# Bluear7878/Remote-Sensing-Vision-Language-Diffusion-Model

Measured on AMD Instinct MI355X. Metric: 512px x8 SR images/sec @50 steps, higher is better.
Workload: dtype f16 / bf16 MFMA operands as hi + lo pairs and triples, f32 accumulation and f32 residual streams (Stage 1: f16 tensors x f16 weight pairs; Stage 2: rsvld_amd.ops.UNET_POLICY; config.precision) -- the composition inside 1e-3 of the reference's CPU path (config.tolerance)

## Files before the change

### remote-sensing-vision-language-diffusion-model_amd/csrc/attention.hip

```cpp
#include "rsvld_common.h"
#include <type_traits>
#include <utility>

namespace {

struct AttnArgs {
    const void* q;
    const void* k;
    const void* v;
    void* out;
    int B, heads, Nq, Nk, D;
    int64_t q_bs, q_ts, k_bs, k_ts, v_bs, v_ts, o_bs, o_ts;
    float scale_log2e;
    unsigned long long* dbg;
};

typedef const __attribute__((address_space(1))) void* gptr_t;
typedef __attribute__((address_space(3))) void* lptr_t;

template <typename F, int... I> __device__ __forceinline__ void static_for_impl(F&& f, std::integer_sequence<int, I...>) {
    (f(std::integral_constant<int, I>{}), ...);
}
template <int N, typename F> __device__ __forceinline__ void static_for(F&& f) {
    static_for_impl(f, std::make_integer_sequence<int, N>{});
}

constexpr float A5_DEFER_LOG2 = 8.0f;

#ifndef A5B_KEYWRAP
#define A5B_KEYWRAP 0
#endif
#ifndef A5B_ABL
#define A5B_ABL 0
#endif
constexpr int A5B_TILE = 32 * 1024;
constexpr int A5B_SMEM = 4 * A5B_TILE;
constexpr int A5B_SMEM_SH = 3 * A5B_TILE;
__host__ __device__ constexpr int a5b_f(int r) { return ((r & 3) << 2) | ((r >> 2) & 3); }
typedef short s16x4 __attribute__((__vector_size__(4 * sizeof(short))));
__device__ __forceinline__ float a5b_halfwave_max(float mx) { return fmaxf(mx, __shfl_xor(mx, 32)); }

template <typename T, bool SH>
__global__ __launch_bounds__(256) void attn_d512b_kernel(AttnArgs p, int keys_per_split, float* part_o, float* part_ml) {
    constexpr int D = 512;
    typedef typename Mfma<T>::v8 v8;
    typedef typename Mfma<T>::v4 v4;
    extern __shared__ __attribute__((aligned(16))) char smem[];

    const int tid = threadIdx.x, lane = tid & 63, w = tid >> 6;
    const int l31 = lane & 31, lh = lane >> 5;
    const int q0 = blockIdx.x * 128 + w * 32;
    const int split = blockIdx.y, nsplit = gridDim.y;
    const int b = blockIdx.z / p.heads, h = blockIdx.z % p.heads;
    const int k_begin = split * keys_per_split;
    const int k_end = min(p.Nk, k_begin + keys_per_split);
    const int nt = (k_end - k_begin + 31) >> 5;
    const T* Qb = (const T*)p.q + (int64_t)b * p.q_bs + (int64_t)h * D;
    const T* Kb = (const T*)p.k + (int64_t)b * p.k_bs + (int64_t)h * D;
    const T* Vb = (const T*)p.v + (int64_t)b * p.v_bs + (int64_t)h * D;

    const int wu = __builtin_amdgcn_readfirstlane(w);
    const uint32_t lds0 = (uint32_t)(uintptr_t)(lptr_t)smem;
    bool abl_dma_on = true;
    auto dma_one = [&](const char* base, uint32_t voff, uint32_t dst) {
        if ((A5B_ABL & 4) && !abl_dma_on) return;
        asm volatile("s_mov_b32 m0, %1\n\ts_nop 0\n\tglobal_load_lds_dwordx4 %0, %2" : : "v"(voff), "s"(dst), "s"(base) : "memory", "m0");
    };
    const int64_t k_rowb = p.k_ts * (int64_t)sizeof(T), v_rowb = p.v_ts * (int64_t)sizeof(T);
    uint32_t kvo[8], vvo[8];
#pragma unroll
    for (int i = 0; i < 8; ++i) {
        kvo[i] = (uint32_t)(i * k_rowb) + (uint32_t)((lane ^ (SH ? a5b_f((wu * 8 + i) & 15) : ((wu * 8 + i) & 15))) << 4);
        vvo[i] = (uint32_t)(i * v_rowb) + (uint32_t)((lane ^ ((i & 3) << 2)) << 4);
    }
    const char* k_tile0 = (const char*)(Kb + (int64_t)(k_begin + wu * 8) * p.k_ts);
    const char* v_tile0 = (const char*)(Vb + (int64_t)(k_begin + wu * 8) * p.v_ts);
    auto dma_kb = [&](int t, int buf, int i) {
        const int r = wu * 8 + i;
        const uint32_t dst = lds0 + buf * A5B_TILE + r * 1024;
        if (k_begin + t * 32 + 32 <= p.Nk) {
            dma_one(k_tile0 + (int64_t)t * 32 * k_rowb, kvo[i], dst);
        } else {
            const int key = min(k_begin + t * 32 + r, p.Nk - 1);
            dma_one((const char*)(Kb + (int64_t)key * p.k_ts), (uint32_t)((lane ^ (SH ? a5b_f(r & 15) : (r & 15))) << 4), dst);
        }
    };
    auto dma_k = [&](int t, int i) { dma_kb(t, t & 1, i); };
    auto dma_v = [&](int t, int i) {
        const int r = wu * 8 + i;
        const uint32_t dst = lds0 + (2 + (t & 1)) * A5B_TILE + r * 1024;
        if (k_begin + t * 32 + 32 <= p.Nk) {
            dma_one(v_tile0 + (int64_t)t * 32 * v_rowb, vvo[i], dst);
        } else {
            const int key = min(k_begin + t * 32 + r, p.Nk - 1);
            dma_one((const char*)(Vb + (int64_t)key * p.v_ts), (uint32_t)((lane ^ ((i & 3) << 2)) << 4), dst);
        }
    };
    auto tw = [](int t) { return A5B_KEYWRAP > 0 ? (t & (A5B_KEYWRAP - 1)) : t; };
    auto dma_kb_fast = [&](int t, int buf, int i) { dma_one(k_tile0 + (int64_t)tw(t) * 32 * k_rowb, kvo[i], lds0 + buf * A5B_TILE + (wu * 8 + i) * 1024); };
    auto dma_k_fast = [&](int t, int i) { dma_kb_fast(t, t & 1, i); };
    auto dma_v_fast = [&](int t, int i) { dma_one(v_tile0 + (int64_t)tw(t) * 32 * v_rowb, vvo[i], lds0 + (2 + (t & 1)) * A5B_TILE + (wu * 8 + i) * 1024); };
    if constexpr (SH) {
#pragma unroll
        for (int i = 0; i < 8; ++i) dma_kb(0, 0, i);
        if (nt > 1) {
#pragma unroll
            for (int i = 0; i < 8; ++i) dma_kb(1, 1, i);
        }
        if (A5B_ABL & 4) {
            if (nt > 2) {
#pragma unroll
                for (int i = 0; i < 8; ++i) dma_kb(2, 2, i);
            }
            abl_dma_on = false;
        }
    } else {
#pragma unroll
    for (int i = 0; i < 8; ++i) { dma_k(0, i); dma_v(0, i); }
    if (nt > 1) {
#pragma unroll
        for (int i = 0; i < 8; ++i) dma_k(1, i);
    }
    }
    if (!SH && (A5B_ABL & 4)) {
        if (nt > 1) {
#pragma unroll
            for (int i = 0; i < 8; ++i) dma_v(1, i);
        }
        abl_dma_on = false;
    }

    const int qrow = q0 + l31;
    v8 qf[32];
#pragma unroll
    for (int ks = 0; ks < 32; ++ks) {
        u32x4 v = {0u, 0u, 0u, 0u};
        if (qrow < p.Nq) v = *(const u32x4*)(Qb + (int64_t)qrow * p.q_ts + ks * 16 + lh * 8);
        qf[ks] = __builtin_bit_cast(v8, v);
    }
    f32x16 oacc[16];
#pragma unroll
    for (int dt = 0; dt < 16; ++dt)
#pragma unroll
        for (int r = 0; r < 16; ++r) oacc[dt][r] = 0.f;
    float m_run = -INFINITY, l_run = 0.f;

    int kbase[8];
#pragma unroll
    for (int c = 0; c < 8; ++c) kbase[c] = l31 * 1024 + (((2 * c + lh) ^ (SH ? a5b_f(l31 & 15) : (l31 & 15))) << 4);
    int vbase[4];
    {
        const int qq = (lane >> 2) & 3, pp = lane & 3, g1 = (lane >> 4) & 1;
#pragma unroll
        for (int f = 0; f < 4; ++f)
            vbase[f] = SH ? (4 * lh + qq) * 1024 + ((f ^ qq) << 6) + (((2 * g1 + (pp >> 1)) ^ lh) << 4) + ((pp & 1) << 3)
                          : 2 * A5B_TILE + (4 * lh + qq) * 1024 + ((f ^ qq) << 6) + ((2 * g1 + (pp >> 1)) << 4) + ((pp & 1) << 3);
    }

    asm volatile("s_waitcnt vmcnt(0)" ::: "memory");
    __syncthreads();

    constexpr int KD = 6;
    static_assert(KD == 6, "A5B_CHAIN's prologue issues 6 reads");
    uint32_t ka[8];
    v8 kfr[KD];
#define A5B_KREAD(slot, ks) \
    asm volatile("ds_read_b128 %0, %1 offset:%2" : "=v"(kfr[slot]) : "v"(ka[(ks) & 7]), "i"(((ks) >> 3) * 256))
#define A5B_STEP(NAME, SACC, ks)                                                                                        \
    asm volatile("s_waitcnt lgkmcnt(%3)\n\t" NAME " %0, %1, %2, %0"                                                      \
                 : "+v"(SACC)                                                                                           \
                 : "v"(kfr[(ks) % KD]), "v"(qf[ks]), "i"(KD - 1 < 31 - (ks) ? KD - 1 : 31 - (ks)));                      \
    if constexpr ((ks) + KD < 32 && !(A5B_ABL & 8)) A5B_KREAD((ks) % KD, (ks) + KD)
#define A5B_STEP4(NAME, SACC, k) \
    A5B_STEP(NAME, SACC, k); A5B_STEP(NAME, SACC, (k) + 1); A5B_STEP(NAME, SACC, (k) + 2); A5B_STEP(NAME, SACC, (k) + 3)
#define A5B_CHAIN(NAME, SACC, KBUF, HOOK)                                                                               \
    _Pragma("unroll") for (int c = 0; c < 8; ++c) ka[c] = lds0 + (uint32_t)((KBUF) * A5B_TILE + kbase[c]);              \
    A5B_KREAD(0, 0); A5B_KREAD(1, 1); A5B_KREAD(2, 2); A5B_KREAD(3, 3); A5B_KREAD(4, 4); A5B_KREAD(5, 5);               \
    asm volatile("s_waitcnt lgkmcnt(%3)\n\t" NAME " %0, %1, %2, 0" : "=&v"(SACC) : "v"(kfr[0]), "v"(qf[0]), "i"(KD - 1)); \
    A5B_KREAD(0, KD);                                                                                                   \
    A5B_STEP(NAME, SACC, 1); A5B_STEP(NAME, SACC, 2); A5B_STEP(NAME, SACC, 3); HOOK(0);                                 \
    A5B_STEP4(NAME, SACC, 4); HOOK(1); A5B_STEP4(NAME, SACC, 8); HOOK(2); A5B_STEP4(NAME, SACC, 12); HOOK(3);           \
    A5B_STEP4(NAME, SACC, 16); HOOK(4); A5B_STEP4(NAME, SACC, 20); HOOK(5); A5B_STEP4(NAME, SACC, 24); HOOK(6);         \
    A5B_STEP4(NAME, SACC, 28); HOOK(7)
#define A5B_MFMA_NAME(T_) (__is_same(T_, f16) ? "f16" : "bf16")
#define A5B_NOHOOK(i)

    f32x16 sacc;
    if constexpr (__is_same(T, f16)) {
        A5B_CHAIN("v_mfma_f32_32x32x16_f16", sacc, 0, A5B_NOHOOK);
    } else {
        A5B_CHAIN("v_mfma_f32_32x32x16_bf16", sacc, 0, A5B_NOHOOK);
    }
    asm volatile("s_nop 15\n\ts_nop 3" : "+v"(sacc));
    __syncthreads();

    int b_pv = 0;
    int t = 0;
    f32x16 sacc2;
#define A5B_STEADY 1
#define A5B_PAIR 1
#define dma_kb_s dma_kb_fast
#define dma_k_s dma_k_fast
#define dma_v_s dma_v_fast
    for (; t + 4 < nt;) {
        {
#define S_CUR sacc
#define S_NXT sacc2
#include "attention_d512_body.inc"
#undef S_CUR
#undef S_NXT
        }
        ++t;
        {
#define S_CUR sacc2
#define S_NXT sacc
#include "attention_d512_body.inc"
#undef S_CUR
#undef S_NXT
        }
        ++t;
    }
#undef dma_kb_s
#undef dma_k_s
#undef dma_v_s
#undef A5B_PAIR
#undef A5B_STEADY
    for (; t < nt; ++t) {
#define A5B_PAIR 0
#define S_CUR sacc
#define S_NXT snext
#define A5B_STEADY 0
#define dma_kb_s dma_kb
#define dma_k_s dma_k
#define dma_v_s dma_v
#include "attention_d512_body.inc"
#undef dma_kb_s
#undef dma_k_s
#undef dma_v_s
#undef A5B_STEADY
#undef S_CUR
#undef S_NXT
#undef A5B_PAIR
    }
#undef A5B_NOHOOK
#undef A5B_MFMA_NAME
#undef A5B_CHAIN
#undef A5B_STEP4
#undef A5B_STEP
#undef A5B_KREAD

    const float l_tot = l_run + __shfl_xor(l_run, 32);
    if (qrow >= p.Nq) return;
    const float inv = 1.0f / l_tot;
    if (nsplit == 1) {
        T* Ob = (T*)p.out + (int64_t)b * p.o_bs + (int64_t)h * D + (int64_t)qrow * p.o_ts;
#pragma unroll
        for (int dt = 0; dt < 16; ++dt)
#pragma unroll
            for (int g = 0; g < 4; ++g) {
                v4 o;
#pragma unroll
                for (int e = 0; e < 4; ++e) o[e] = (T)(oacc[dt][4 * g + e] * inv);
                *(v4*)(Ob + dt * 32 + 8 * g + 4 * lh) = o;
            }
    } else {
        const int64_t row = ((int64_t)split * gridDim.z + blockIdx.z) * p.Nq + qrow;
        float* Po = part_o + row * D;
#pragma unroll
        for (int dt = 0; dt < 16; ++dt)
#pragma unroll
            for (int g = 0; g < 4; ++g) {
                f32x4 o;
#pragma unroll
                for (int e = 0; e < 4; ++e) o[e] = oacc[dt][4 * g + e] * inv;
                *(f32x4*)(Po + dt * 32 + 8 * g + 4 * lh) = o;
            }
        if (lh == 0) {
            part_ml[row * 2] = m_run;
            part_ml[row * 2 + 1] = l_tot;
        }
    }
}

template <typename T>
__global__ __launch_bounds__(128) void attn_combine_kernel(AttnArgs p, int nsplit, const float* part_o, const float* part_ml) {
    constexpr int D = 512;
    typedef typename Mfma<T>::v4 v4;
    const int qrow = blockIdx.x, bh = blockIdx.y;
    const int b = bh / p.heads, h = bh % p.heads;
    const int64_t nrows = (int64_t)gridDim.y * p.Nq;
    float mmax = -INFINITY;
    for (int i = 0; i < nsplit; ++i) mmax = fmaxf(mmax, part_ml[((int64_t)i * nrows + (int64_t)bh * p.Nq + qrow) * 2]);
    float wsum = 0.f;
    f32x4 acc = {0.f, 0.f, 0.f, 0.f};
    for (int i = 0; i < nsplit; ++i) {
        const int64_t row = (int64_t)i * nrows + (int64_t)bh * p.Nq + qrow;
        const float wi = part_ml[row * 2 + 1] * __builtin_amdgcn_exp2f(part_ml[row * 2] - mmax);
        const f32x4 o = *(const f32x4*)(part_o + row * D + threadIdx.x * 4);
        acc += o * wi;
        wsum += wi;
    }
    const float inv = 1.0f / wsum;
    v4 o;
#pragma unroll
    for (int e = 0; e < 4; ++e) o[e] = (T)(acc[e] * inv);
    *(v4*)((T*)p.out + (int64_t)b * p.o_bs + (int64_t)h * D + (int64_t)qrow * p.o_ts + threadIdx.x * 4) = o;
}

#include "attention_d512d.inc"

}

namespace {

constexpr int A6B_TILE = 64 * 128;
#ifndef A6B_ABL
#define A6B_ABL 0
#endif
#ifndef A6B_STAMP
#define A6B_STAMP 0
#endif
__device__ __forceinline__ unsigned long long a6b_stamp() {
    unsigned long long t;
    __builtin_amdgcn_sched_barrier(0);
    asm volatile("s_memtime %0\n\ts_waitcnt lgkmcnt(0)" : "=s"(t) :: "memory");
    __builtin_amdgcn_sched_barrier(0);
    return t;
}

__device__ __forceinline__ float a6b_add(float a, float b) { return a + b; }

template <typename T>
__device__ __forceinline__ void a6_store_o(char* wbuf, const f32x16 (&oacc)[2], float inv, int q0, int lane, const AttnArgs& p, int b, int h) {
    typedef typename Mfma<T>::v4 v4;
    const int l31 = lane & 31, lh = lane >> 5;
    T* Ob = (T*)p.out + (int64_t)b * p.o_bs + (int64_t)h * 64;
#pragma unroll
    for (int dt = 0; dt < 2; ++dt)
#pragma unroll
        for (int g = 0; g < 4; ++g) {
            v4 o;
#pragma unroll
            for (int e = 0; e < 4; ++e) o[e] = (T)(oacc[dt][4 * g + e] * inv);
// ... 404 lines not shown
```

### remote-sensing-vision-language-diffusion-model_amd/csrc/attention_d512d.inc

```
constexpr int A5D_P_OFF = 4 * A5B_TILE;
constexpr int A5D_PBUF = 4 * 2 * 64 * 16;
constexpr int A5D_A_OFF = A5D_P_OFF + 2 * A5D_PBUF;
constexpr int A5D_L_OFF = A5D_A_OFF + 2 * 512;
constexpr int A5D_SMEM = A5D_L_OFF + 512;

template <typename T>
__global__ __launch_bounds__(256) void attn_d512d_kernel(AttnArgs p, int keys_per_split, float* part_o, float* part_ml) {
    constexpr int D = 512;
    typedef typename Mfma<T>::v8 v8;
    typedef typename Mfma<T>::v4 v4;
    extern __shared__ __attribute__((aligned(16))) char smem[];

    const int tid = threadIdx.x, lane = tid & 63, w = tid >> 6;
    const int l31 = lane & 31, lh = lane >> 5;
    const int q0 = blockIdx.x * 128 + w * 32;
    const int split = blockIdx.y, nsplit = gridDim.y;
    const int b = blockIdx.z / p.heads, h = blockIdx.z % p.heads;
    const int k_begin = split * keys_per_split;
    const int k_end = min(p.Nk, k_begin + keys_per_split);
    const int nt = (k_end - k_begin + 31) >> 5;
    const T* Qb = (const T*)p.q + (int64_t)b * p.q_bs + (int64_t)h * D;
    const T* Xb = (const T*)p.k + (int64_t)b * p.k_bs + (int64_t)h * D;

    const int wu = __builtin_amdgcn_readfirstlane(w);
    const uint32_t lds0 = (uint32_t)(uintptr_t)(lptr_t)smem;
    auto dma_one = [&](const char* base, uint32_t voff, uint32_t dst) {
        asm volatile("s_mov_b32 m0, %1\n\ts_nop 0\n\tglobal_load_lds_dwordx4 %0, %2" : : "v"(voff), "s"(dst), "s"(base) : "memory", "m0");
    };
    const int64_t x_rowb = p.k_ts * (int64_t)sizeof(T);
    const uint32_t lane16 = (uint32_t)lane << 4;
    const char* x_tile0 = (const char*)(Xb + (int64_t)(k_begin + wu * 8) * p.k_ts);
    auto dma_x = [&](int t, int i) {
        const int r = wu * 8 + i;
        const uint32_t dst = lds0 + (t & 3) * A5B_TILE + r * 1024;
        if (k_begin + t * 32 + 32 <= p.Nk) {
            dma_one(x_tile0 + (int64_t)(t * 32 + i) * x_rowb, lane16 ^ (uint32_t)(a5b_f(r & 15) << 4), dst);
        } else {
            const int key = min(k_begin + t * 32 + r, p.Nk - 1);
            dma_one((const char*)(Xb + (int64_t)key * p.k_ts), lane16 ^ (uint32_t)(a5b_f(r & 15) << 4), dst);
        }
    };
    auto dma_x_fast = [&](int t, int i) {
        const int r = wu * 8 + i;
        dma_one(x_tile0 + (int64_t)(t * 32 + i) * x_rowb, lane16 ^ (uint32_t)(a5b_f(r & 15) << 4), lds0 + (t & 3) * A5B_TILE + r * 1024);
    };
#pragma unroll
    for (int i = 0; i < 8; ++i) dma_x(0, i);
    if (nt > 1) {
#pragma unroll
        for (int i = 0; i < 8; ++i) dma_x(1, i);
    }
    if (nt > 2) {
#pragma unroll
        for (int i = 0; i < 8; ++i) dma_x(2, i);
    }

    const int qrow = q0 + l31;
    v8 qf[32];
#pragma unroll
    for (int ks = 0; ks < 32; ++ks) {
        u32x4 v = {0u, 0u, 0u, 0u};
        if (qrow < p.Nq) v = *(const u32x4*)(Qb + (int64_t)qrow * p.q_ts + ks * 16 + lh * 8);
        qf[ks] = __builtin_bit_cast(v8, v);
    }
    f32x16 oacc[4][4];
#pragma unroll
    for (int dt = 0; dt < 4; ++dt)
#pragma unroll
        for (int j = 0; j < 4; ++j)
#pragma unroll
            for (int r = 0; r < 16; ++r) oacc[dt][j][r] = 0.f;
    float m_run = -INFINITY, l_run = 0.f;

    const uint32_t kb = l31 * 1024 + ((lh ^ a5b_f(l31 & 15)) << 4);
    int vbase[4];
    {
        const int qq = (lane >> 2) & 3, pp = lane & 3, g1 = (lane >> 4) & 1;
#pragma unroll
        for (int f = 0; f < 4; ++f) vbase[f] = (4 * lh + qq) * 1024 + ((f ^ qq) << 6) + (((2 * g1 + (pp >> 1)) ^ lh) << 4) + ((pp & 1) << 3) + wu * 256;
    }
    auto vread = [&](int buf, int f, int s2) {
        const int off = buf * A5B_TILE + vbase[f] + (16 * s2) * 1024;
        const s16x4 lo = __builtin_amdgcn_ds_read_tr16_b64_v4i16((__attribute__((address_space(3))) s16x4*)(smem + off));
        const s16x4 hi = __builtin_amdgcn_ds_read_tr16_b64_v4i16((__attribute__((address_space(3))) s16x4*)(smem + ((off ^ 32) + 8 * 1024)));
        typedef short s16x8 __attribute__((__vector_size__(8 * sizeof(short))));
        return __builtin_bit_cast(v8, (s16x8)__builtin_shufflevector(lo, hi, 0, 1, 2, 3, 4, 5, 6, 7));
    };
    const int p_own = A5D_P_OFF + wu * 2048 + lane * 16, a_own = A5D_A_OFF + l31 * 16 + wu * 4;
    int p_oth[3], a_oth[3];
#pragma unroll
    for (int j = 1; j < 4; ++j) {
        p_oth[j - 1] = A5D_P_OFF + ((wu + j) & 3) * 2048 + lane * 16;
        a_oth[j - 1] = A5D_A_OFF + l31 * 16 + ((wu + j) & 3) * 4;
    }

    asm volatile("s_waitcnt vmcnt(0)" ::: "memory");
    __syncthreads();

    constexpr int KD = 6;
    uint32_t ka[8];
    v8 kfr[KD];
#define A5D_KREAD(slot, ks) \
    asm volatile("ds_read_b128 %0, %1 offset:%2" : "=v"(kfr[slot]) : "v"(ka[(ks) & 7]), "i"(((ks) >> 3) * 256))
#define A5D_STEP(NAME, SACC, ks)                                                                                        \
    asm volatile("s_waitcnt lgkmcnt(%3)\n\t" NAME " %0, %1, %2, %0"                                                      \
                 : "+v"(SACC)                                                                                           \
                 : "v"(kfr[(ks) % KD]), "v"(qf[ks]), "i"(KD - 1 < 31 - (ks) ? KD - 1 : 31 - (ks)));                      \
    if constexpr ((ks) + KD < 32) A5D_KREAD((ks) % KD, (ks) + KD)
#define A5D_STEP4(NAME, SACC, k) \
    A5D_STEP(NAME, SACC, k); A5D_STEP(NAME, SACC, (k) + 1); A5D_STEP(NAME, SACC, (k) + 2); A5D_STEP(NAME, SACC, (k) + 3)
#define A5D_CHAIN(NAME, SACC, KBUF, HOOK)                                                                               \
    _Pragma("unroll") for (int c = 0; c < 8; ++c) ka[c] = lds0 + (((KBUF) * A5B_TILE + kb) ^ (c << 5));         \
    A5D_KREAD(0, 0); A5D_KREAD(1, 1); A5D_KREAD(2, 2); A5D_KREAD(3, 3); A5D_KREAD(4, 4); A5D_KREAD(5, 5);               \
    asm volatile("s_waitcnt lgkmcnt(%3)\n\t" NAME " %0, %1, %2, 0" : "=&v"(SACC) : "v"(kfr[0]), "v"(qf[0]), "i"(KD - 1)); \
    A5D_KREAD(0, KD);                                                                                                   \
    A5D_STEP(NAME, SACC, 1); A5D_STEP(NAME, SACC, 2); A5D_STEP(NAME, SACC, 3); HOOK(0);                                 \
    A5D_STEP4(NAME, SACC, 4); HOOK(1); A5D_STEP4(NAME, SACC, 8); HOOK(2); A5D_STEP4(NAME, SACC, 12); HOOK(3);           \
    A5D_STEP4(NAME, SACC, 16); HOOK(4); A5D_STEP4(NAME, SACC, 20); HOOK(5); A5D_STEP4(NAME, SACC, 24); HOOK(6);         \
    A5D_STEP4(NAME, SACC, 28); HOOK(7)
#define A5D_NOHOOK(i)

    f32x16 sacc;
    if constexpr (__is_same(T, f16)) {
        A5D_CHAIN("v_mfma_f32_32x32x16_f16", sacc, 0, A5D_NOHOOK);
    } else {
        A5D_CHAIN("v_mfma_f32_32x32x16_bf16", sacc, 0, A5D_NOHOOK);
    }
    asm volatile("s_nop 15\n\ts_nop 3" : "+v"(sacc));

    int t = 0;
    f32x16 sacc2;
#define A5D_STEADY 1
#define A5D_PAIR 1
    for (; t + 5 < nt;) {
        {
#define S_CUR sacc
#define S_NXT sacc2
#include "attention_d512d_body.inc"
#undef S_CUR
#undef S_NXT
        }
        ++t;
        {
#define S_CUR sacc2
#define S_NXT sacc
#include "attention_d512d_body.inc"
#undef S_CUR
#undef S_NXT
        }
        ++t;
    }
#undef A5D_PAIR
#undef A5D_STEADY
    for (; t < nt; ++t) {
#define A5D_PAIR 0
#define A5D_STEADY 0
#define S_CUR sacc
#define S_NXT snext
#include "attention_d512d_body.inc"
#undef S_NXT
#undef S_CUR
#undef A5D_STEADY
#undef A5D_PAIR
    }
#undef A5D_NOHOOK
#undef A5D_CHAIN
#undef A5D_STEP4
#undef A5D_STEP
#undef A5D_KREAD

    const float l_tot = l_run + __shfl_xor(l_run, 32);
    *(float*)(smem + A5D_L_OFF + l31 * 16 + wu * 4) = l_tot;
    __syncthreads();
    float inv[4];
    inv[0] = 1.0f / l_tot;
#pragma unroll
    for (int j = 1; j < 4; ++j) inv[j] = 1.0f / *(const float*)(smem + A5D_L_OFF + l31 * 16 + ((wu + j) & 3) * 4);
#pragma unroll
    for (int j = 0; j < 4; ++j) {
        const int qr = blockIdx.x * 128 + ((wu + j) & 3) * 32 + l31;
        if (qr >= p.Nq) continue;
        if (nsplit == 1) {
            T* Ob = (T*)p.out + (int64_t)b * p.o_bs + (int64_t)h * D + (int64_t)qr * p.o_ts + wu * 128;
#pragma unroll
            for (int dt = 0; dt < 4; ++dt)
#pragma unroll
                for (int g = 0; g < 4; ++g) {
                    v4 o;
#pragma unroll
                    for (int e = 0; e < 4; ++e) o[e] = (T)(oacc[dt][j][4 * g + e] * inv[j]);
                    *(v4*)(Ob + dt * 32 + 8 * g + 4 * lh) = o;
                }
        } else {
            const int64_t row = ((int64_t)split * gridDim.z + blockIdx.z) * p.Nq + qr;
            float* Po = part_o + row * D + wu * 128;
#pragma unroll
            for (int dt = 0; dt < 4; ++dt)
#pragma unroll
                for (int g = 0; g < 4; ++g) {
                    f32x4 o;
#pragma unroll
                    for (int e = 0; e < 4; ++e) o[e] = oacc[dt][j][4 * g + e] * inv[j];
                    *(f32x4*)(Po + dt * 32 + 8 * g + 4 * lh) = o;
                }
            if (j == 0 && lh == 0) {
                part_ml[row * 2] = m_run;
                part_ml[row * 2 + 1] = l_tot;
            }
        }
    }
}
```

### remote-sensing-vision-language-diffusion-model_amd/csrc/attention_d512d_body.inc

```
        const bool more = A5D_STEADY ? true : t + 1 < nt;
        const int b_pv = t & 3, pb = (t & 1) * A5D_PBUF, ab = (t & 1) * 512;

        float mx = -INFINITY, alpha = 1.0f, rs = 0.f;
        bool need = false;
        v8 pf[2];
        auto sm = [&](int part) {
            if (part == 0) {
                if (!A5D_STEADY && k_begin + (t + 1) * 32 > k_end) {
#pragma unroll
                    for (int r = 0; r < 16; ++r) {
                        const int kv = k_begin + t * 32 + (r & 3) + 8 * (r >> 2) + 4 * lh;
                        if (kv >= k_end) S_CUR[r] = -INFINITY;
                    }
                }
#pragma unroll
                for (int r = 0; r < 16; ++r) mx = fmaxf(mx, S_CUR[r]);
                asm volatile("" : "+v"(S_CUR), "+v"(mx));
            } else if (part == 1) {
                mx = a5b_halfwave_max(mx) * p.scale_log2e;
                need = mx > m_run + A5_DEFER_LOG2;
                if (need) {
                    alpha = __builtin_amdgcn_exp2f(m_run - mx);
                    m_run = mx;
                }
                asm volatile("" : "+v"(alpha), "+v"(m_run));
            } else if (part >= 2 && part <= 5) {
                const int r0 = 4 * (part - 2);
#pragma unroll
                for (int r = r0; r < r0 + 4; ++r) {
                    S_CUR[r] = __builtin_amdgcn_exp2f(__builtin_fmaf(S_CUR[r], p.scale_log2e, -m_run));
                    rs += S_CUR[r];
                }
                asm volatile("" : "+v"(S_CUR[r0]), "+v"(S_CUR[r0 + 1]), "+v"(S_CUR[r0 + 2]), "+v"(S_CUR[r0 + 3]), "+v"(rs));
            } else if (part == 6) {
                l_run = l_run * alpha + rs;
#pragma unroll
                for (int s2 = 0; s2 < 2; ++s2)
#pragma unroll
                    for (int j = 0; j < 8; ++j) pf[s2][j] = (T)S_CUR[8 * s2 + j];
                asm volatile("" : "+v"(pf[0]), "+v"(pf[1]), "+v"(l_run));
            }
        };
#if !A5D_PAIR
        f32x16 snext;
#endif
        if (more) {
#define A5D_HOOK(i) \
    sm(i);          \
    __builtin_amdgcn_sched_barrier(0)
            if constexpr (__is_same(T, f16)) {
                A5D_CHAIN("v_mfma_f32_32x32x16_f16", S_NXT, ((t + 1) & 3), A5D_HOOK);
            } else {
                A5D_CHAIN("v_mfma_f32_32x32x16_bf16", S_NXT, ((t + 1) & 3), A5D_HOOK);
            }
#undef A5D_HOOK
        } else {
#pragma unroll
            for (int i = 0; i < 7; ++i) sm(i);
        }

        *(v8*)(smem + pb + p_own) = pf[0];
        *(v8*)(smem + pb + p_own + 1024) = pf[1];
        *(float*)(smem + ab + a_own) = alpha;
        v8 vfr[2][4];
#pragma unroll
        for (int s2 = 0; s2 < 2; ++s2)
#pragma unroll
            for (int f = 0; f < 4; ++f) vfr[s2][f] = vread(b_pv, f, s2);
        asm volatile("s_waitcnt vmcnt(0)" ::: "memory");
        __syncthreads();

        v8 pfo[2][3];
        float al[3];
#pragma unroll
        for (int s2 = 0; s2 < 2; ++s2)
#pragma unroll
            for (int j = 0; j < 3; ++j) pfo[s2][j] = *(const v8*)(smem + pb + p_oth[j] + 1024 * s2);
#pragma unroll
        for (int j = 0; j < 3; ++j) al[j] = *(const float*)(smem + ab + a_oth[j]);

#define A5D_RESCALE(J, A)                                                                                                  \
    _Pragma("unroll") for (int dt = 0; dt < 4; ++dt)                                                                       \
    _Pragma("unroll") for (int r = 0; r < 16; ++r) {                                                                       \
        float x = oacc[dt][J][r], tmp;                                                                                     \
        asm volatile("v_accvgpr_read_b32 %1, %0\n\tv_mul_f32 %1, %1, %2\n\ts_nop 0\n\tv_accvgpr_write_b32 %0, %1\n\ts_nop 1" \
                     : "+a"(x), "=&v"(tmp)                                                                                 \
                     : "v"(A));                                                                                            \
        oacc[dt][J][r] = x;                                                                                                \
    }
        if (__builtin_expect(__any(need), 0)) {
            asm volatile("s_nop 15\n\ts_nop 3" ::: "memory");
            A5D_RESCALE(0, alpha)
        }
        __builtin_amdgcn_sched_barrier(0);
#pragma unroll
        for (int s2 = 0; s2 < 2; ++s2)
#pragma unroll
            for (int f = 0; f < 4; ++f) {
                oacc[f][0] = Mfma<T>::mma(vfr[s2][f], pf[s2], oacc[f][0]);
                __builtin_amdgcn_sched_barrier(0);
            }
        if (__builtin_expect(__any(al[0] != 1.0f || al[1] != 1.0f || al[2] != 1.0f), 0)) {
            asm volatile("s_nop 15\n\ts_nop 3" ::: "memory");
            A5D_RESCALE(1, al[0])
            A5D_RESCALE(2, al[1])
            A5D_RESCALE(3, al[2])
        }
#undef A5D_RESCALE
        __builtin_amdgcn_sched_barrier(0);
#pragma unroll
        for (int n = 0; n < 24; ++n) {
            const int s2 = n / 12, f = (n / 3) & 3, j = n % 3;
            oacc[f][j + 1] = Mfma<T>::mma(vfr[s2][f], pfo[s2][j], oacc[f][j + 1]);
            if (n % 3 == 2) {
                if (A5D_STEADY) {
                    dma_x_fast(t + 3, n / 3);
                } else if (t + 3 < nt) {
                    dma_x(t + 3, n / 3);
                }
            }
            __builtin_amdgcn_sched_barrier(0);
        }
#if !A5D_PAIR
        if (more) S_CUR = S_NXT;
#endif
```

Baseline: 0.01348.

## Spread softmax work across QK MFMA chain and hoist max into PV phase

Restructures the online-softmax placement in the d512 attention kernel. The row max and the rescale decision move out of the per-tile softmax and are computed either after the QK chain or interleaved with the own-P PV MFMAs. Exp, conversion and sum work is issued one step at a time after each QK MFMA, and the cross-half max uses permlane32_swap instead of a shuffle. LDS addresses are split into lane and scalar wave parts so they can use SGPR offsets. The aim is to hide softmax VALU latency under MFMA issue, at the cost of more complex scheduling, register pressure, and macro-selected variants.

```diff
diff --git a/remote-sensing-vision-language-diffusion-model_amd/csrc/attention.hip b/remote-sensing-vision-language-diffusion-model_amd/csrc/attention.hip
--- a/remote-sensing-vision-language-diffusion-model_amd/csrc/attention.hip
+++ b/remote-sensing-vision-language-diffusion-model_amd/csrc/attention.hip
@@ -33,12 +33,21 @@
 #ifndef A5B_ABL
 #define A5B_ABL 0
 #endif
+#ifndef A5D_ABL
+#define A5D_ABL 0
+#endif
 constexpr int A5B_TILE = 32 * 1024;
 constexpr int A5B_SMEM = 4 * A5B_TILE;
 constexpr int A5B_SMEM_SH = 3 * A5B_TILE;
 __host__ __device__ constexpr int a5b_f(int r) { return ((r & 3) << 2) | ((r >> 2) & 3); }
 typedef short s16x4 __attribute__((__vector_size__(4 * sizeof(short))));
 __device__ __forceinline__ float a5b_halfwave_max(float mx) { return fmaxf(mx, __shfl_xor(mx, 32)); }
+__device__ __forceinline__ void a5d_halfwave_swap(float mx, float& lo, float& hi) {
+    const uint32_t mb = __builtin_bit_cast(uint32_t, mx);
+    const auto sw = __builtin_amdgcn_permlane32_swap(mb, mb, false, false);
+    lo = __builtin_bit_cast(float, (uint32_t)sw[0]);
+    hi = __builtin_bit_cast(float, (uint32_t)sw[1]);
+}
 
 template <typename T, bool SH>
 __global__ __launch_bounds__(256) void attn_d512b_kernel(AttnArgs p, int keys_per_split, float* part_o, float* part_ml) {
diff --git a/remote-sensing-vision-language-diffusion-model_amd/csrc/attention_d512d.inc b/remote-sensing-vision-language-diffusion-model_amd/csrc/attention_d512d.inc
--- a/remote-sensing-vision-language-diffusion-model_amd/csrc/attention_d512d.inc
+++ b/remote-sensing-vision-language-diffusion-model_amd/csrc/attention_d512d.inc
@@ -1,3 +1,6 @@
+#ifndef A5D_PLACE
+#define A5D_PLACE 7
+#endif
 constexpr int A5D_P_OFF = 4 * A5B_TILE;
 constexpr int A5D_PBUF = 4 * 2 * 64 * 16;
 constexpr int A5D_A_OFF = A5D_P_OFF + 2 * A5D_PBUF;
@@ -86,13 +89,18 @@
         typedef short s16x8 __attribute__((__vector_size__(8 * sizeof(short))));
         return __builtin_bit_cast(v8, (s16x8)__builtin_shufflevector(lo, hi, 0, 1, 2, 3, 4, 5, 6, 7));
     };
-    const int p_own = A5D_P_OFF + wu * 2048 + lane * 16, a_own = A5D_A_OFF + l31 * 16 + wu * 4;
+    const int p_lane = lane * 16, a_lane = l31 * 16;
+    const int p_own = A5D_P_OFF + wu * 2048, a_own = A5D_A_OFF + wu * 4;
     int p_oth[3], a_oth[3];
 #pragma unroll
     for (int j = 1; j < 4; ++j) {
-        p_oth[j - 1] = A5D_P_OFF + ((wu + j) & 3) * 2048 + lane * 16;
-        a_oth[j - 1] = A5D_A_OFF + l31 * 16 + ((wu + j) & 3) * 4;
-    }
+        p_oth[j - 1] = A5D_P_OFF + ((wu + j) & 3) * 2048;
+        a_oth[j - 1] = A5D_A_OFF + ((wu + j) & 3) * 4;
+    }
+    auto xaddr = [&](int lane_part, int wave_part) __attribute__((always_inline)) {
+        asm volatile("" : "+s"(wave_part));
+        return smem + (lane_part + wave_part);
+    };
 
     asm volatile("s_waitcnt vmcnt(0)" ::: "memory");
     __syncthreads();
@@ -102,23 +110,63 @@
     v8 kfr[KD];
 #define A5D_KREAD(slot, ks) \
     asm volatile("ds_read_b128 %0, %1 offset:%2" : "=v"(kfr[slot]) : "v"(ka[(ks) & 7]), "i"(((ks) >> 3) * 256))
-#define A5D_STEP(NAME, SACC, ks)                                                                                        \
+#define A5D_STEP(NAME, SACC, ks, HOOK)                                                                                  \
     asm volatile("s_waitcnt lgkmcnt(%3)\n\t" NAME " %0, %1, %2, %0"                                                      \
                  : "+v"(SACC)                                                                                           \
                  : "v"(kfr[(ks) % KD]), "v"(qf[ks]), "i"(KD - 1 < 31 - (ks) ? KD - 1 : 31 - (ks)));                      \
-    if constexpr ((ks) + KD < 32) A5D_KREAD((ks) % KD, (ks) + KD)
-#define A5D_STEP4(NAME, SACC, k) \
-    A5D_STEP(NAME, SACC, k); A5D_STEP(NAME, SACC, (k) + 1); A5D_STEP(NAME, SACC, (k) + 2); A5D_STEP(NAME, SACC, (k) + 3)
+    if constexpr ((ks) + KD < 32) A5D_KREAD((ks) % KD, (ks) + KD);                                                      \
+    HOOK(ks)
+#define A5D_STEP4(NAME, SACC, k, HOOK) \
+    A5D_STEP(NAME, SACC, k, HOOK); A5D_STEP(NAME, SACC, (k) + 1, HOOK); A5D_STEP(NAME, SACC, (k) + 2, HOOK); A5D_STEP(NAME, SACC, (k) + 3, HOOK)
 #define A5D_CHAIN(NAME, SACC, KBUF, HOOK)                                                                               \
     _Pragma("unroll") for (int c = 0; c < 8; ++c) ka[c] = lds0 + (((KBUF) * A5B_TILE + kb) ^ (c << 5));         \
     A5D_KREAD(0, 0); A5D_KREAD(1, 1); A5D_KREAD(2, 2); A5D_KREAD(3, 3); A5D_KREAD(4, 4); A5D_KREAD(5, 5);               \
     asm volatile("s_waitcnt lgkmcnt(%3)\n\t" NAME " %0, %1, %2, 0" : "=&v"(SACC) : "v"(kfr[0]), "v"(qf[0]), "i"(KD - 1)); \
-    A5D_KREAD(0, KD);                                                                                                   \
-    A5D_STEP(NAME, SACC, 1); A5D_STEP(NAME, SACC, 2); A5D_STEP(NAME, SACC, 3); HOOK(0);                                 \
-    A5D_STEP4(NAME, SACC, 4); HOOK(1); A5D_STEP4(NAME, SACC, 8); HOOK(2); A5D_STEP4(NAME, SACC, 12); HOOK(3);           \
-    A5D_STEP4(NAME, SACC, 16); HOOK(4); A5D_STEP4(NAME, SACC, 20); HOOK(5); A5D_STEP4(NAME, SACC, 24); HOOK(6);         \
-    A5D_STEP4(NAME, SACC, 28); HOOK(7)
+    A5D_KREAD(0, KD); HOOK(0);                                                                                          \
+    A5D_STEP(NAME, SACC, 1, HOOK); A5D_STEP(NAME, SACC, 2, HOOK); A5D_STEP(NAME, SACC, 3, HOOK);                        \
+    A5D_STEP4(NAME, SACC, 4, HOOK); A5D_STEP4(NAME, SACC, 8, HOOK); A5D_STEP4(NAME, SACC, 12, HOOK);                    \
+    A5D_STEP4(NAME, SACC, 16, HOOK); A5D_STEP4(NAME, SACC, 20, HOOK); A5D_STEP4(NAME, SACC, 24, HOOK);                  \
+    A5D_STEP4(NAME, SACC, 28, HOOK)
 #define A5D_NOHOOK(i)
+
+    auto mx4 = [&](f32x16& S, int tile, int i, float& mx, bool masked) __attribute__((always_inline)) {
+        if (masked && k_begin + (tile + 1) * 32 > k_end) {
+#pragma unroll
+            for (int r = 4 * i; r < 4 * i + 4; ++r) {
+                const int kv = k_begin + tile * 32 + (r & 3) + 8 * (r >> 2) + 4 * lh;
+                if (kv >= k_end) S[r] = -INFINITY;
+            }
+        }
+#pragma unroll
+        for (int r = 4 * i; r < 4 * i + 4; ++r) mx = fmaxf(mx, S[r]);
+        asm volatile("" : "+v"(mx));
+    };
+    auto mx_half0 = [&](float mx, float& lo, float& hi) __attribute__((always_inline)) {
+        if (A5D_PLACE & 1) {
+            a5d_halfwave_swap(mx, lo, hi);
+        } else {
+            lo = mx;
+            hi = __shfl_xor(mx, 32);
+        }
+        asm volatile("" : "+v"(lo), "+v"(hi));
+    };
+    auto mx_half1 = [&](float& mx, float lo, float hi) __attribute__((always_inline)) {
+        mx = fmaxf(lo, hi);
+        asm volatile("" : "+v"(mx));
+    };
+    float alpha = 1.0f, a_new = 1.0f;
+    bool need = false;
+    auto mx_dec0 = [&](float& mx) __attribute__((always_inline)) {
+        mx *= p.scale_log2e;
+        need = mx > m_run + A5_DEFER_LOG2;
+        a_new = __builtin_amdgcn_exp2f(m_run - mx);
+        asm volatile("" : "+v"(mx), "+v"(a_new));
+    };
+    auto mx_dec1 = [&](float mx) __attribute__((always_inline)) {
+        alpha = need ? a_new : 1.0f;
+        m_run = need ? mx : m_run;
+        asm volatile("" : "+v"(alpha), "+v"(m_run));
+    };
 
     f32x16 sacc;
     if constexpr (__is_same(T, f16)) {
@@ -127,6 +175,16 @@
         A5D_CHAIN("v_mfma_f32_32x32x16_bf16", sacc, 0, A5D_NOHOOK);
     }
     asm volatile("s_nop 15\n\ts_nop 3" : "+v"(sacc));
+    if ((A5D_PLACE & 2) && !(A5D_ABL & 1)) {
+        float mx = -INFINITY;
+#pragma unroll
+        for (int i = 0; i < 4; ++i) mx4(sacc, 0, i, mx, true);
+        float lo, hi;
+        mx_half0(mx, lo, hi);
+        mx_half1(mx, lo, hi);
+        mx_dec0(mx);
+        mx_dec1(mx);
+    }
 
     int t = 0;
     f32x16 sacc2;
diff --git a/remote-sensing-vision-language-diffusion-model_amd/csrc/attention_d512d_body.inc b/remote-sensing-vision-language-diffusion-model_amd/csrc/attention_d512d_body.inc
--- a/remote-sensing-vision-language-diffusion-model_amd/csrc/attention_d512d_body.inc
+++ b/remote-sensing-vision-language-diffusion-model_amd/csrc/attention_d512d_body.inc
@@ -1,45 +1,61 @@
         const bool more = A5D_STEADY ? true : t + 1 < nt;
         const int b_pv = t & 3, pb = (t & 1) * A5D_PBUF, ab = (t & 1) * 512;
-
-        float mx = -INFINITY, alpha = 1.0f, rs = 0.f;
-        bool need = false;
-        v8 pf[2];
-        auto sm = [&](int part) {
+        float rs = 0.f;
+#if !(A5D_PLACE & 2)
+        float mx = -INFINITY, m_lo, m_hi;
+        alpha = 1.0f;
+        need = false;
+#endif
+        u32x2 pk[4];
+        auto el = [&](int r) __attribute__((always_inline)) {
+            S_CUR[r] = __builtin_amdgcn_exp2f(__builtin_fmaf(S_CUR[r], p.scale_log2e, -m_run));
+            rs += S_CUR[r];
+            asm volatile("" : "+v"(S_CUR[r]), "+v"(rs));
+        };
+        auto cv = [&](int i) __attribute__((always_inline)) {
+            v4 h;
+#pragma unroll
+            for (int j = 0; j < 4; ++j) h[j] = (T)S_CUR[4 * i + j];
+            pk[i] = __builtin_bit_cast(u32x2, h);
+            asm volatile("" : "+v"(pk[i]));
+        };
+        auto lr = [&]() __attribute__((always_inline)) {
+            l_run = l_run * alpha + rs;
+            asm volatile("" : "+v"(l_run));
+        };
+        auto sm = [&](int s) __attribute__((always_inline)) {
+            if (A5D_ABL & 1) {
+                if (s >= 27 && s < 31) cv(s - 27);
+                return;
+            }
+#if A5D_PLACE & 4
+            constexpr int e0 = (A5D_PLACE & 2) ? 0 : 6;
+#if !(A5D_PLACE & 2)
+            if (s < 4) mx4(S_CUR, t, s, mx, !A5D_STEADY);
+            else if (s == 4) mx_half0(mx, m_lo, m_hi);
+            else if (s == 5) { mx_half1(mx, m_lo, m_hi); mx_dec0(mx); mx_dec1(mx); }
+#endif
+            if (s >= e0 && s < e0 + 16) el(s - e0);
+            else if (s == e0 + 16) lr();
+            else if (s >= 27 && s < 31) cv(s - 27);
+#else
+            if ((s & 3) != 3) return;
+            const int part = s >> 2;
+#if !(A5D_PLACE & 2)
             if (part == 0) {
-                if (!A5D_STEADY && k_begin + (t + 1) * 32 > k_end) {
 #pragma unroll
-                    for (int r = 0; r < 16; ++r) {
-                        const int kv = k_begin + t * 32 + (r & 3) + 8 * (r >> 2) + 4 * lh;
-                        if (kv >= k_end) S_CUR[r] = -INFINITY;
-                    }
-                }
+                for (int i = 0; i < 4; ++i) mx4(S_CUR, t, i, mx, !A5D_STEADY);
+            } else if (part == 1) { mx_half0(mx, m_lo, m_hi); mx_half1(mx, m_lo, m_hi); mx_dec0(mx); mx_dec1(mx); }
+#endif
+            if (part >= 2 && part <= 5) {
 #pragma unroll
-                for (int r = 0; r < 16; ++r) mx = fmaxf(mx, S_CUR[r]);
-                asm volatile("" : "+v"(S_CUR), "+v"(mx));
-            } else if (part == 1) {
-                mx = a5b_halfwave_max(mx) * p.scale_log2e;
-                need = mx > m_run + A5_DEFER_LOG2;
-                if (need) {
-                    alpha = __builtin_amdgcn_exp2f(m_run - mx);
-                    m_run = mx;
-                }
-                asm volatile("" : "+v"(alpha), "+v"(m_run));
-            } else if (part >= 2 && part <= 5) {
-                const int r0 = 4 * (part - 2);
+                for (int r = 4 * (part - 2); r < 4 * (part - 2) + 4; ++r) el(r);
+            } else if (part == 6) {
+                lr();
 #pragma unroll
-                for (int r = r0; r < r0 + 4; ++r) {
-                    S_CUR[r] = __builtin_amdgcn_exp2f(__builtin_fmaf(S_CUR[r], p.scale_log2e, -m_run));
-                    rs += S_CUR[r];
-                }
-                asm volatile("" : "+v"(S_CUR[r0]), "+v"(S_CUR[r0 + 1]), "+v"(S_CUR[r0 + 2]), "+v"(S_CUR[r0 + 3]), "+v"(rs));
-            } else if (part == 6) {
-                l_run = l_run * alpha + rs;
-#pragma unroll
-                for (int s2 = 0; s2 < 2; ++s2)
-#pragma unroll
-                    for (int j = 0; j < 8; ++j) pf[s2][j] = (T)S_CUR[8 * s2 + j];
-                asm volatile("" : "+v"(pf[0]), "+v"(pf[1]), "+v"(l_run));
+                for (int i = 0; i < 4; ++i) cv(i);
             }
+#endif
         };
 #if !A5D_PAIR
         f32x16 snext;
@@ -56,12 +72,16 @@
 #undef A5D_HOOK
         } else {
 #pragma unroll
-            for (int i = 0; i < 7; ++i) sm(i);
+            for (int i = 0; i < 32; ++i) sm(i);
         }
+        v8 pf[2];
+        pf[0] = __builtin_bit_cast(v8, (u32x4)__builtin_shufflevector(pk[0], pk[1], 0, 1, 2, 3));
+        pf[1] = __builtin_bit_cast(v8, (u32x4)__builtin_shufflevector(pk[2], pk[3], 0, 1, 2, 3));
 
-        *(v8*)(smem + pb + p_own) = pf[0];
-        *(v8*)(smem + pb + p_own + 1024) = pf[1];
-        *(float*)(smem + ab + a_own) = alpha;
+        char* const p_dst = xaddr(p_lane, pb + p_own);
+        *(v8*)p_dst = pf[0];
+        *(v8*)(p_dst + 1024) = pf[1];
+        *(float*)xaddr(a_lane, ab + a_own) = alpha;
         v8 vfr[2][4];
 #pragma unroll
         for (int s2 = 0; s2 < 2; ++s2)
@@ -73,11 +93,13 @@
         v8 pfo[2][3];
         float al[3];
 #pragma unroll
-        for (int s2 = 0; s2 < 2; ++s2)
+        for (int j = 0; j < 3; ++j) {
+            const char* const p_src = xaddr(p_lane, pb + p_oth[j]);
+            pfo[0][j] = *(const v8*)p_src;
+            pfo[1][j] = *(const v8*)(p_src + 1024);
+        }
 #pragma unroll
-            for (int j = 0; j < 3; ++j) pfo[s2][j] = *(const v8*)(smem + pb + p_oth[j] + 1024 * s2);
-#pragma unroll
-        for (int j = 0; j < 3; ++j) al[j] = *(const float*)(smem + ab + a_oth[j]);
+        for (int j = 0; j < 3; ++j) al[j] = *(const float*)xaddr(a_lane, ab + a_oth[j]);
 
 #define A5D_RESCALE(J, A)                                                                                                  \
     _Pragma("unroll") for (int dt = 0; dt < 4; ++dt)                                                                       \
@@ -93,11 +115,24 @@
             A5D_RESCALE(0, alpha)
         }
         __builtin_amdgcn_sched_barrier(0);
+#if A5D_PLACE & 2
+        float mx_n = -INFINITY, m_lo_n, m_hi_n;
+#endif
 #pragma unroll
         for (int s2 = 0; s2 < 2; ++s2)
 #pragma unroll
             for (int f = 0; f < 4; ++f) {
                 oacc[f][0] = Mfma<T>::mma(vfr[s2][f], pf[s2], oacc[f][0]);
+#if A5D_PLACE & 2
+                if (A5D_STEADY && !(A5D_ABL & 1)) {
+                    const int g = 4 * s2 + f;
+                    if (g < 4) mx4(S_NXT, t + 1, g, mx_n, false);
+                    else if (g == 4) mx_half0(mx_n, m_lo_n, m_hi_n);
+                    else if (g == 5) mx_half1(mx_n, m_lo_n, m_hi_n);
+                    else if (g == 6) mx_dec0(mx_n);
+                    else mx_dec1(mx_n);
+                }
+#endif
                 __builtin_amdgcn_sched_barrier(0);
             }
         if (__builtin_expect(__any(al[0] != 1.0f || al[1] != 1.0f || al[2] != 1.0f), 0)) {
@@ -122,5 +157,18 @@
             __builtin_amdgcn_sched_barrier(0);
         }
 #if !A5D_PAIR
-        if (more) S_CUR = S_NXT;
+        if (more) {
+            S_CUR = S_NXT;
+#if A5D_PLACE & 2
+            if (!(A5D_ABL & 1)) {
+                float mx = -INFINITY, lo, hi;
+#pragma unroll
+                for (int i = 0; i < 4; ++i) mx4(S_CUR, t + 1, i, mx, true);
+                mx_half0(mx, lo, hi);
+                mx_half1(mx, lo, hi);
+                mx_dec0(mx);
+                mx_dec1(mx);
+            }
 #endif
+        }
+#endif
```

After: 0.01348. About the same (-0.1%).
